# pkorus/neural-imaging

Hardware: AMD Instinct MI355X
Metric: patches/s (fwd+bwd) ISP->JPEG->FAN @256^2 (higher is better)
Workload: dtype bf16; 1 GPU; c4 = train_manipulation UNet->[native,sharpen:1,resample:50,gaussian:0.83,jpeg:80]->dJPEG(QF80,soft)->FAN, ds none, trainable nip+fan, lambda_nip 0.1; raw_patch=128, batch_per_gpu=64, global_batch=64, parallelism=dp1, world_size=1, hip_graph=False

## Files before the change

neural-imaging_amd/csrc/conv_bf16_ring.h:

```cpp
#pragma once
#include "conv_bf16.h"

namespace {

typedef unsigned int r_u32x4 __attribute__((ext_vector_type(4)));
__device__ __forceinline__ void glds16(r_u32x4 rsrc, unsigned lds_addr, unsigned voff, int soff) {
    unsigned keep;
    asm volatile("s_mov_b32 %0, m0\n\ts_mov_b32 m0, %1\n\ts_nop 0\n\tbuffer_load_dwordx4 %2, %3, %4 offen lds\n\ts_mov_b32 m0, %0"
                 : "=&s"(keep) : "s"(lds_addr), "v"(voff), "s"(rsrc), "s"(soff) : "memory");
}
__device__ __forceinline__ void dma_wait() { asm volatile("s_waitcnt vmcnt(0)" ::: "memory"); }
template <int N>
__device__ __forceinline__ void dma_wait_leave() { asm volatile("s_waitcnt vmcnt(%0)" ::"n"(N) : "memory"); }

#ifndef NIMG_RING_ABLATE
#define NIMG_RING_ABLATE 0
#endif

template <int TN, int NW = 4, int KS = 5>
struct RingGeom {
    static constexpr int NI = TN / 32, MI = NI == 1 ? 4 : 8 / NI;
    static constexpr int NT = 64 * NW;
    static constexpr int TH = 2 * NW * MI, TW = 16, THH = TH + KS - 1, TWH = TW + KS - 1;
    static constexpr int NPIXH = THH * TWH, AP = (NPIXH * 2 + NT - 1) / NT;
    static constexpr int PLSZ = THH * 32;
    static constexpr int ABUF = 2 * PLSZ;
    static constexpr bool ADBL = TN == 128;
    static constexpr int SLOT = KS * TN * 2;
    static constexpr int PIECES = KS * NI, NPW = (PIECES + NW - 1) / NW;
#ifdef NIMG_RING_SLOTS2
    static constexpr int NSLOT = 2;
#else
    static constexpr int NSLOT = (NW == 8 && KS == 5) ? 3 : 2;
#endif
    static constexpr size_t LDS_TILES = (size_t)(NSLOT * SLOT + (ADBL ? 2 : 1) * ABUF) * sizeof(uint4);
    static constexpr size_t LDS_EPI = (size_t)NW * 32 * (TN + EPI_PAD) * sizeof(float);
    static constexpr size_t LDS = LDS_TILES > LDS_EPI ? LDS_TILES : LDS_EPI;
};

template <int TN, bool UNP, int NW = 4, int KS = 5>
__global__ __launch_bounds__(64 * NW, NW == 8 ? 2 : (TN == 32 ? 3 : 2)) void conv5_ring_kernel(const ConvParamsB p) {
    using G = RingGeom<TN, NW, KS>;
    static_assert(KS == 5 || (KS == 3 && !UNP && NW == 4), "kernel size 3: plain input, four waves");
    constexpr int NT = G::NT;
    constexpr int NI = G::NI, MI = G::MI, TH = G::TH, TW = G::TW, TWH = G::TWH, NPIXH = G::NPIXH, AP = G::AP;
    constexpr int PLSZ = G::PLSZ, ABUF = G::ABUF, SLOT = G::SLOT;
    extern __shared__ __attribute__((aligned(16))) unsigned char smem_raw[];
    uint4* sB = reinterpret_cast<uint4*>(smem_raw);
    uint4* sA = sB + G::NSLOT * SLOT;
    const unsigned sB_addr = (unsigned)(unsigned long)(__attribute__((address_space(3))) unsigned char*)smem_raw;
    const int tid = threadIdx.x, lane = tid & 63;
    const int wave = __builtin_amdgcn_readfirstlane(tid >> 6);
    const int Cout = p.O1;
    const int cot = Cout / TN;
    int bid = xcd_order(blockIdx.x);
    const int co0 = (bid % cot) * TN;
    bid /= cot;
    const int tiles = p.tiles_y * p.tiles_x;
    const int tile = bid % tiles, grp = bid / tiles;
    const int ty0 = (tile / p.tiles_x) * TH, tx0 = (tile % p.tiles_x) * TW;
    const int iy0 = ty0 - p.pad_t, ix0 = tx0 - p.pad_l;
    const int half = lane >> 5;

    int abase[MI];
#pragma unroll
    for (int mi = 0; mi < MI; ++mi) {
        const int P = (wave * MI + mi) * 32 + (lane & 31);
        abase[mi] = half * PLSZ + (P / TW) * 32 + (P % TW);
    }
    const int bbase = (lane & 31) * 2 + (half ^ (((lane & 31) >> 3) & 1));
    f32x16 acc[MI][NI];
#pragma unroll
    for (int mi = 0; mi < MI; ++mi)
#pragma unroll
        for (int ni = 0; ni < NI; ++ni)
#pragma unroll
            for (int j = 0; j < 16; ++j) acc[mi][ni][j] = 0.0f;

    typedef unsigned int u32x4 __attribute__((ext_vector_type(4)));
    typedef unsigned int u32x2k __attribute__((ext_vector_type(2)));
    unsigned aoff[AP], upos[UNP ? AP : 1];
    int adst[AP];
#pragma unroll
    for (int q = 0; q < AP; ++q) {
        const int item = tid + q * NT, pix = item >> 1;
        int gy = iy0 + pix / TWH, gx = ix0 + pix % TWH;
        const bool ok = (item < NPIXH * 2) & (grp < p.N) & map_coord(gy, p.H, p.pad_mode) & map_coord(gx, p.W, p.pad_mode);
        int apix;
        if constexpr (UNP) {
            apix = (grp * (p.H >> 1) + (gy >> 1)) * (p.W >> 1) + (gx >> 1);
            upos[q] = (unsigned)(((gy & 1) << 1) | (gx & 1));
        } else {
            apix = (grp * p.H + gy) * p.W + gx;
        }
        aoff[q] = ok ? (unsigned)((apix * p.C1 + (tid & 1) * 8) * 2) : 0x80000000u;
        adst[q] = (tid & 1) * PLSZ + (pix / TWH) * 32 + pix % TWH;
    }
    const __amdgpu_buffer_rsrc_t ra = __builtin_amdgcn_make_buffer_rsrc(
        const_cast<float*>(p.in1), 0, (int)(((long)p.N * p.H * p.W * p.C1 * 2) >> (UNP ? 2 : 0)), 0x00020000);
    const unsigned long wb_addr = (unsigned long)p.wb;
    const r_u32x4 rb = {(unsigned)wb_addr, (unsigned)(wb_addr >> 32) & 0xffffu,
                        (unsigned)((long)(p.CinP >> 4) * KS * KS * 16 * Cout * 2), 0x00020000u};
    const __amdgpu_buffer_rsrc_t rk = __builtin_amdgcn_make_buffer_rsrc(
        const_cast<unsigned char*>(UNP ? p.in_idx : reinterpret_cast<const unsigned char*>(p.in1)), 0,
        (int)(((long)p.N * p.H * p.W * p.C1) >> 2), 0x00020000);
    uint4 preA[AP];
    u32x2k preK[UNP ? AP : 1];
    auto fetchA = [&](int c0) {
#pragma unroll
        for (int q = 0; q < AP; ++q) {
            const u32x4 v = __builtin_amdgcn_raw_buffer_load_b128(ra, aoff[q], c0 * 2, 0);
            preA[q] = *reinterpret_cast<const uint4*>(&v);
            if constexpr (UNP)
                preK[q] = __builtin_amdgcn_raw_buffer_load_b64(rk, aoff[q] >= 0x80000000u ? 0x80000000u : aoff[q] >> 1, c0, 0);
        }
    };
    auto commitA = [&](int buf) {
#pragma unroll
        for (int q = 0; q < AP; ++q) {
            if (tid + q * NT < NPIXH * 2) {
                uint4 v = preA[q];
                if constexpr (UNP) v = unp_route(v, preK[q][0], preK[q][1], upos[q]);
                sA[buf + adst[q]] = v;
            }
        }
    };
    const unsigned bvoff = (unsigned)(((co0 + (lane >> 1)) * 16 + (((lane & 1) ^ ((lane >> 4) & 1)) * 8)) * 2);
    auto gldsB = [&](int chunk, int ky, int slot) {
#pragma unroll
        for (int j = 0; j < G::NPW; ++j) {
            const int k = wave + NW * j;
            if (G::PIECES % NW == 0 || k < G::PIECES) {
                const int soff = ((chunk * KS * KS + ky * KS + k / NI) * Cout + (k % NI) * 32) * 32;
                glds16(rb, sB_addr + (unsigned)((slot * SLOT + k * 64) * 16), bvoff, soff);
            }
        }
    };
    const int chunks = p.C1 >> 4;
    gldsB(0, 0, 0);
    if constexpr (G::NSLOT == 3) gldsB(0, 1, 1);
    fetchA(0);
    commitA(0);
    dma_wait();
    __syncthreads();
    constexpr int ABL = NIMG_RING_ABLATE;
    bf16x8 a0[MI], b0[NI];
    if constexpr (ABL & 8) {
#pragma unroll
        for (int mi = 0; mi < MI; ++mi) { const uint4 v = sA[abase[mi]]; a0[mi] = *reinterpret_cast<const bf16x8*>(&v); }
#pragma unroll
        for (int ni = 0; ni < NI; ++ni) { const uint4 v = sB[bbase + ni * 64]; b0[ni] = *reinterpret_cast<const bf16x8*>(&v); }
    }
    if constexpr (G::NSLOT == 3) {
        static_assert(G::ADBL, "the three-slot ring is written for the double-buffered input tile");
        constexpr int NLO = G::PIECES / NW, NREM = G::PIECES % NW;
        constexpr int NA = AP * (UNP ? 2 : 1);
        int s0 = 0;
        for (int c = 0; c < chunks; ++c) {
            const int ab = (c & 1) * ABUF;
            const bool more = c + 1 < chunks;
#pragma unroll
            for (int ky = 0; ky < 5; ++ky) {
                const int slot = (s0 + ky) % 3, slot2 = (s0 + ky + 2) % 3;
                if (ky == 2 && more) commitA(ab ^ ABUF);
                const bool issue = ky < 3 || more;
                if (ky < 3) gldsB(c, ky + 2, slot2);
                else if (more) gldsB(c + 1, ky - 3, slot2);
                if (ky == 0 && more) fetchA((c + 1) * 16);
                const uint4* sBs = sB + slot * SLOT + bbase;
#pragma unroll
                for (int kx = 0; kx < 5; ++kx) {
                    bf16x8 a[MI], b[NI];
#pragma unroll
                    for (int mi = 0; mi < MI; ++mi) {
                        const uint4 v = sA[ab + abase[mi] + ky * 32 + kx];
                        a[mi] = *reinterpret_cast<const bf16x8*>(&v);
                    }
#pragma unroll
                    for (int ni = 0; ni < NI; ++ni) {
                        const uint4 v = sBs[(kx * TN + ni * 32) * 2];
                        b[ni] = *reinterpret_cast<const bf16x8*>(&v);
                    }
#pragma unroll
                    for (int mi = 0; mi < MI; ++mi)
#pragma unroll
                        for (int ni = 0; ni < NI; ++ni)
                            acc[mi][ni] = __builtin_amdgcn_mfma_f32_32x32x16_bf16(a[mi], b[ni], acc[mi][ni], 0, 0, 0);
                }
                if (!issue) dma_wait();
                else if (ky < 2 && more) {
                    if (NREM && wave < NREM) dma_wait_leave<NLO + 1 + NA>();
                    else dma_wait_leave<NLO + NA>();
                } else {
                    if (NREM && wave < NREM) dma_wait_leave<NLO + 1>();
                    else dma_wait_leave<NLO>();
                }
                asm volatile("s_waitcnt lgkmcnt(0)\n\ts_barrier" ::: "memory");
            }
            s0 = (s0 + 2) % 3;
        }
    } else
    for (int c = 0; c < chunks; ++c) {
        const int ab = G::ADBL ? (c & 1) * ABUF : 0;
        const bool more = c + 1 < chunks;
#pragma unroll
        for (int ky = 0; ky < KS; ++ky) {
            const int slot = (c + ky) & 1;
            if constexpr (!(ABL & 1)) {
                if (ky < KS - 1) gldsB(c, ky + 1, slot ^ 1);
                else if (more) gldsB(c + 1, 0, slot ^ 1);
            }
            if constexpr (!(ABL & 2)) if (ky == 0 && more) fetchA((c + 1) * 16);
            const uint4* sBs = sB + slot * SLOT + bbase;
#pragma unroll
            for (int kx = 0; kx < KS; ++kx) {
                bf16x8 a[MI], b[NI];
#pragma unroll
                for (int mi = 0; mi < MI; ++mi) {
                    if constexpr (ABL & 8) { a[mi] = a0[mi]; continue; }
                    const uint4 v = sA[ab + abase[mi] + ky * 32 + kx];
                    a[mi] = *reinterpret_cast<const bf16x8*>(&v);
                }
#pragma unroll
                for (int ni = 0; ni < NI; ++ni) {
                    if constexpr (ABL & 8) { b[ni] = b0[ni]; continue; }
                    const uint4 v = sBs[(kx * TN + ni * 32) * 2];
                    b[ni] = *reinterpret_cast<const bf16x8*>(&v);
                }
#pragma unroll
                for (int mi = 0; mi < MI; ++mi)
#pragma unroll
                    for (int ni = 0; ni < NI; ++ni)
                        acc[mi][ni] = __builtin_amdgcn_mfma_f32_32x32x16_bf16(a[mi], b[ni], acc[mi][ni], 0, 0, 0);
            }
            if constexpr (!(ABL & 2)) if (G::ADBL && ky == KS - 1 && more) commitA(ab ^ ABUF);
            if constexpr (!(ABL & 4)) {
                dma_wait();
                __syncthreads();
            }
            if constexpr (!(ABL & 2)) if (!G::ADBL && ky == KS - 1 && more) {
                commitA(0);
                if constexpr (!(ABL & 4)) __syncthreads();
            }
        }
    }
    if constexpr (ABL & 4) { dma_wait(); __syncthreads(); }
    if constexpr (ABL & 16) {
        float sacc = 0.f;
#pragma unroll
        for (int mi = 0; mi < MI; ++mi)
#pragma unroll
            for (int ni = 0; ni < NI; ++ni)
#pragma unroll
                for (int j = 0; j < 16; ++j) sacc += acc[mi][ni][j];
        if (sacc == 123.456f) p.out1[0] = sacc;
        return;
    }
    if constexpr (KS == 3) {
        conv_epilogue_vec<3, TH, TW, 1, MI, NI>(acc, p, smem_raw, wave, lane, wave, 0, co0, Cout, ty0, tx0, grp, 0,
                                                epi_bias_preload<NI>(p, lane, 0, co0, Cout));
        return;
    }
    float* elds = reinterpret_cast<float*>(smem_raw) + wave * (32 * (NI * 32 + EPI_PAD));
    if (p.pool_out) {
        const int Hp = p.Hout >> 1, Wp = p.Wout >> 1;
        const float al = p.act == 1 ? p.alpha : 1.0f;
        if (p.flags & NIMG_BF16_OUT) {
#pragma unroll
            for (int mi = 0; mi < MI; ++mi) {
                const int py = (ty0 >> 1) + wave * MI + mi;
                pool_in_regs8<NI>(acc[mi], elds, lane, al,
                    [&](int c) { return p.bias ? p.bias[co0 + c] : 0.f; },
                    [&](int pc, int c, float4 lo, float4 hi, uint2 k) {
                        const int px = (tx0 >> 1) + pc;
                        if (grp >= p.N || py >= Hp || px >= Wp) return;
                        const long o = (((long)grp * Hp + py) * Wp + px) * Cout + co0 + c;
                        const float f[8] = {lo.x, lo.y, lo.z, lo.w, hi.x, hi.y, hi.z, hi.w};
                        const bf16x8 pk = pack8(f);
                        *reinterpret_cast<bf16x8*>(reinterpret_cast<__bf16*>(p.pool_out) + o) = pk;
                        if (p.pool_idx) *reinterpret_cast<uint2*>(p.pool_idx + o) = k;
                        if (p.pool_sign) {
                            const uint4 pw = __builtin_bit_cast(uint4, pk);
                            const unsigned sb = bf16x2_positive(pw.x) | (bf16x2_positive(pw.y) << 1) | (bf16x2_positive(pw.z) << 2) |
                                                (bf16x2_positive(pw.w) << 3);
                            p.pool_sign[o >> 3] = (unsigned char)sign_bits_interleave(sb);
                        }
                    });
            }
            return;
        }
#pragma unroll
        for (int mi = 0; mi < MI; ++mi) {
            const int py = (ty0 >> 1) + wave * MI + mi;
            pool_in_regs<NI>(acc[mi], elds, lane, al,
                [&](int c) { return p.bias ? p.bias[co0 + c] : 0.f; },
                [&](int pc, int c, float4 v, uchar4 k) {
                    const int co = co0 + c, px = (tx0 >> 1) + pc;
                    if (grp >= p.N || py >= Hp || px >= Wp) return;
                    const long o = (((long)grp * Hp + py) * Wp + px) * Cout + co;
                    if (p.flags & NIMG_BF16_OUT) store4_bf16(p.pool_out, o, v);
                    else *reinterpret_cast<float4*>(p.pool_out + o) = v;
                    if (p.pool_idx) *reinterpret_cast<uchar4*>(p.pool_idx + o) = k;
                });
        }
        return;
    }
    if ((p.flags & NIMG_BF16_OUT) && (!p.act1 || (p.flags & NIMG_BF16_MASK))) {
#pragma unroll
        for (int mi = 0; mi < MI; ++mi) {
            epilogue_via_lds8<NI>(acc[mi], elds, lane, [&](int row, int c, float4 lo, float4 hi) {
                const int P = (wave * MI + mi) * 32 + row;
                const int oy = ty0 + P / TW, ox = tx0 + P % TW;
                if (grp >= p.N || oy >= p.Hout || ox >= p.Wout) return;
                const long o = (((long)grp * p.Hout + oy) * p.Wout + ox) * Cout + co0 + c;
                float f[8] = {lo.x, lo.y, lo.z, lo.w, hi.x, hi.y, hi.z, hi.w};
                if (p.bias) {
#pragma unroll
                    for (int e = 0; e < 8; ++e) f[e] += p.bias[co0 + c + e];
                }
                if (p.act == 1) {
#pragma unroll
                    for (int e = 0; e < 8; ++e) f[e] = lrelu(f[e], p.alpha);
                }
                if (p.act_sign) {
                    const unsigned sb = p.act_sign[o >> 3];
#pragma unroll
                    for (int e = 0; e < 8; ++e) f[e] *= ((sb >> e) & 1u) ? 1.0f : p.alpha;
                } else if (p.act1) {
                    const bf16x8 m = *reinterpret_cast<const bf16x8*>(reinterpret_cast<const __bf16*>(p.act1) + o);
#pragma unroll
                    for (int e = 0; e < 8; ++e) f[e] *= (float)m[e] > 0.f ? 1.0f : p.alpha;
                }
                *reinterpret_cast<bf16x8*>(reinterpret_cast<__bf16*>(p.out1) + o) = pack8(f);
            });
        }
        return;
    }
#pragma unroll
    for (int mi = 0; mi < MI; ++mi) {
        epilogue_via_lds<NI, false>(acc[mi], elds, lane, [&](int row, int c, float4 v) {
            const int co = co0 + c;
            const int P = (wave * MI + mi) * 32 + row;
            const int oy = ty0 + P / TW, ox = tx0 + P % TW;
            if (grp >= p.N || oy >= p.Hout || ox >= p.Wout) return;
            const long o = (((long)grp * p.Hout + oy) * p.Wout + ox) * Cout + co;
            if (p.bias) {
                const float4 b = *reinterpret_cast<const float4*>(p.bias + co);
                v.x += b.x; v.y += b.y; v.z += b.z; v.w += b.w;
            }
            if (p.act == 1) {
                v.x = lrelu(v.x, p.alpha); v.y = lrelu(v.y, p.alpha); v.z = lrelu(v.z, p.alpha); v.w = lrelu(v.w, p.alpha);
            }
            if (p.act1) {
                const float4 m = (p.flags & NIMG_BF16_MASK) ? load4_bf16(p.act1, o) : *reinterpret_cast<const float4*>(p.act1 + o);
                v.x *= m.x > 0.f ? 1.0f : p.alpha; v.y *= m.y > 0.f ? 1.0f : p.alpha;
                v.z *= m.z > 0.f ? 1.0f : p.alpha; v.w *= m.w > 0.f ? 1.0f : p.alpha;
            }
            if (p.flags & NIMG_BF16_OUT) store4_bf16(p.out1, o, v);
            else *reinterpret_cast<float4*>(p.out1 + o) = v;
        });
    }
}

template <int TN, int NW = 4, int KS = 5>
int launch_conv5_ring(const ConvParamsB& p, hipStream_t stream) {
    using G = RingGeom<TN, NW, KS>;
    if constexpr (NW == 4 && TN == 128 && KS == 5) {
        static const bool nw8 = getenv("NIMG_RING_NW8") != nullptr;
        if (nw8 && p.Hout % 32 == 0) return launch_conv5_ring<TN, 8>(p, stream);
    }
    ConvParamsB q = p;
    q.tiles_y = cdiv(p.Hout, G::TH);
    q.tiles_x = cdiv(p.Wout, G::TW);
    const long blocks = (long)(p.O1 / TN) * q.tiles_y * q.tiles_x * p.N;
    auto kern = conv5_ring_kernel<TN, false, NW, KS>;
    if constexpr (KS == 5) { if (p.in_idx) kern = conv5_ring_kernel<TN, true, NW, KS>; }
    (void)hipFuncSetAttribute((const void*)kern, hipFuncAttributeMaxDynamicSharedMemorySize, (int)G::LDS);
    hipLaunchKernelGGL(kern, dim3((unsigned)blocks), dim3(G::NT), G::LDS, stream, q);
    NIMG_CHECK_LAUNCH();
    return NIMG_OK;
}

}
```

Baseline: 8073 patches/s.

## Stage unpooled input per pooling window and keep A fragments in registers across rows

For the max-unpool input path, each load item now covers a whole 2x2 pooling window. One global fetch of values and indices is routed to four LDS positions, where before each pixel was fetched separately. For the TN=32 unpool case, A fragments read at even ky are kept in registers and reused by later even rows, which cuts LDS reads. It also adds a launch-time guard that rejects unpool inputs whose padding or sizes do not align with the pooling windows. The cost is extra register pressure, and unsupported configurations now return an error.

```diff
diff --git a/neural-imaging_amd/csrc/conv_bf16_ring.h b/neural-imaging_amd/csrc/conv_bf16_ring.h
--- a/neural-imaging_amd/csrc/conv_bf16_ring.h
+++ b/neural-imaging_amd/csrc/conv_bf16_ring.h
@@ -22,7 +22,6 @@
     static constexpr int NI = TN / 32, MI = NI == 1 ? 4 : 8 / NI;
     static constexpr int NT = 64 * NW;
     static constexpr int TH = 2 * NW * MI, TW = 16, THH = TH + KS - 1, TWH = TW + KS - 1;
-    static constexpr int NPIXH = THH * TWH, AP = (NPIXH * 2 + NT - 1) / NT;
     static constexpr int PLSZ = THH * 32;
     static constexpr int ABUF = 2 * PLSZ;
     static constexpr bool ADBL = TN == 128;
@@ -43,7 +42,7 @@
     using G = RingGeom<TN, NW, KS>;
     static_assert(KS == 5 || (KS == 3 && !UNP && NW == 4), "kernel size 3: plain input, four waves");
     constexpr int NT = G::NT;
-    constexpr int NI = G::NI, MI = G::MI, TH = G::TH, TW = G::TW, TWH = G::TWH, NPIXH = G::NPIXH, AP = G::AP;
+    constexpr int NI = G::NI, MI = G::MI, TH = G::TH, TW = G::TW, TWH = G::TWH;
     constexpr int PLSZ = G::PLSZ, ABUF = G::ABUF, SLOT = G::SLOT;
     extern __shared__ __attribute__((aligned(16))) unsigned char smem_raw[];
     uint4* sB = reinterpret_cast<uint4*>(smem_raw);
@@ -79,22 +78,20 @@
 
     typedef unsigned int u32x4 __attribute__((ext_vector_type(4)));
     typedef unsigned int u32x2k __attribute__((ext_vector_type(2)));
-    unsigned aoff[AP], upos[UNP ? AP : 1];
-    int adst[AP];
-#pragma unroll
-    for (int q = 0; q < AP; ++q) {
-        const int item = tid + q * NT, pix = item >> 1;
-        int gy = iy0 + pix / TWH, gx = ix0 + pix % TWH;
-        const bool ok = (item < NPIXH * 2) & (grp < p.N) & map_coord(gy, p.H, p.pad_mode) & map_coord(gx, p.W, p.pad_mode);
-        int apix;
-        if constexpr (UNP) {
-            apix = (grp * (p.H >> 1) + (gy >> 1)) * (p.W >> 1) + (gx >> 1);
-            upos[q] = (unsigned)(((gy & 1) << 1) | (gx & 1));
-        } else {
-            apix = (grp * p.H + gy) * p.W + gx;
-        }
+    constexpr int SW = UNP ? 2 : 1;
+    static_assert(G::THH % SW == 0 && TWH % SW == 0 && TH % SW == 0 && TW % SW == 0, "a halo of whole pooling windows");
+    constexpr int CW = TWH / SW, NITEM = (G::THH / SW) * CW * 2, AQ = (NITEM + NT - 1) / NT;
+    unsigned aoff[AQ];
+    int adst[AQ];
+#pragma unroll
+    for (int q = 0; q < AQ; ++q) {
+        const int item = tid + q * NT, cell = item >> 1;
+        const int hy = (cell / CW) * SW, hx = (cell % CW) * SW;
+        int gy = iy0 + hy, gx = ix0 + hx;
+        const bool ok = (item < NITEM) & (grp < p.N) & map_coord(gy, p.H, p.pad_mode) & map_coord(gx, p.W, p.pad_mode);
+        const int apix = UNP ? (grp * (p.H >> 1) + (gy >> 1)) * (p.W >> 1) + (gx >> 1) : (grp * p.H + gy) * p.W + gx;
         aoff[q] = ok ? (unsigned)((apix * p.C1 + (tid & 1) * 8) * 2) : 0x80000000u;
-        adst[q] = (tid & 1) * PLSZ + (pix / TWH) * 32 + pix % TWH;
+        adst[q] = (tid & 1) * PLSZ + hy * 32 + hx;
     }
     const __amdgpu_buffer_rsrc_t ra = __builtin_amdgcn_make_buffer_rsrc(
         const_cast<float*>(p.in1), 0, (int)(((long)p.N * p.H * p.W * p.C1 * 2) >> (UNP ? 2 : 0)), 0x00020000);
@@ -104,11 +101,11 @@
     const __amdgpu_buffer_rsrc_t rk = __builtin_amdgcn_make_buffer_rsrc(
         const_cast<unsigned char*>(UNP ? p.in_idx : reinterpret_cast<const unsigned char*>(p.in1)), 0,
         (int)(((long)p.N * p.H * p.W * p.C1) >> 2), 0x00020000);
-    uint4 preA[AP];
-    u32x2k preK[UNP ? AP : 1];
+    uint4 preA[AQ];
+    u32x2k preK[UNP ? AQ : 1];
     auto fetchA = [&](int c0) {
 #pragma unroll
-        for (int q = 0; q < AP; ++q) {
+        for (int q = 0; q < AQ; ++q) {
             const u32x4 v = __builtin_amdgcn_raw_buffer_load_b128(ra, aoff[q], c0 * 2, 0);
             preA[q] = *reinterpret_cast<const uint4*>(&v);
             if constexpr (UNP)
@@ -117,11 +114,15 @@
     };
     auto commitA = [&](int buf) {
 #pragma unroll
-        for (int q = 0; q < AP; ++q) {
-            if (tid + q * NT < NPIXH * 2) {
-                uint4 v = preA[q];
-                if constexpr (UNP) v = unp_route(v, preK[q][0], preK[q][1], upos[q]);
-                sA[buf + adst[q]] = v;
+        for (int q = 0; q < AQ; ++q) {
+            if (tid + q * NT < NITEM) {
+                if constexpr (UNP) {
+#pragma unroll
+                    for (int pos = 0; pos < 4; ++pos)
+                        sA[buf + adst[q] + (pos >> 1) * 32 + (pos & 1)] = unp_route(preA[q], preK[q][0], preK[q][1], (unsigned)pos);
+                } else {
+                    sA[buf + adst[q]] = preA[q];
+                }
             }
         }
     };
@@ -144,6 +145,7 @@
     dma_wait();
     __syncthreads();
     constexpr int ABL = NIMG_RING_ABLATE;
+    constexpr bool KEEP = TN == 32 && UNP && KS == 5 && !ABL;
     bf16x8 a0[MI], b0[NI];
     if constexpr (ABL & 8) {
 #pragma unroll
@@ -154,7 +156,7 @@
     if constexpr (G::NSLOT == 3) {
         static_assert(G::ADBL, "the three-slot ring is written for the double-buffered input tile");
         constexpr int NLO = G::PIECES / NW, NREM = G::PIECES % NW;
-        constexpr int NA = AP * (UNP ? 2 : 1);
+        constexpr int NA = AQ * (UNP ? 2 : 1);
         int s0 = 0;
         for (int c = 0; c < chunks; ++c) {
             const int ab = (c & 1) * ABUF;
@@ -203,6 +205,7 @@
     for (int c = 0; c < chunks; ++c) {
         const int ab = G::ADBL ? (c & 1) * ABUF : 0;
         const bool more = c + 1 < chunks;
+        bf16x8 ak[KEEP ? MI + KS / 2 : 1][KS];
 #pragma unroll
         for (int ky = 0; ky < KS; ++ky) {
             const int slot = (c + ky) & 1;
@@ -218,8 +221,11 @@
 #pragma unroll
                 for (int mi = 0; mi < MI; ++mi) {
                     if constexpr (ABL & 8) { a[mi] = a0[mi]; continue; }
+                    const bool kept = KEEP && !(ky & 1);
+                    if (kept && ky >= 2 && mi < MI - 1) { a[mi] = ak[mi + ky / 2][kx]; continue; }
                     const uint4 v = sA[ab + abase[mi] + ky * 32 + kx];
                     a[mi] = *reinterpret_cast<const bf16x8*>(&v);
+                    if (kept) ak[mi + ky / 2][kx] = a[mi];
                 }
 #pragma unroll
                 for (int ni = 0; ni < NI; ++ni) {
@@ -369,6 +375,7 @@
         static const bool nw8 = getenv("NIMG_RING_NW8") != nullptr;
         if (nw8 && p.Hout % 32 == 0) return launch_conv5_ring<TN, 8>(p, stream);
     }
+    if (p.in_idx && (p.pad_t != 2 || p.pad_l != 2 || p.pad_mode != 0 || (p.H & 1) || (p.W & 1))) return NIMG_ERR_ARG;
     ConvParamsB q = p;
     q.tiles_y = cdiv(p.Hout, G::TH);
     q.tiles_x = cdiv(p.Wout, G::TW);
```

Result: no change. 8128 patches/s, median of 6 (+0.7%).
